# WeiZhang1988/YDORBSLAM

Measured on AMD Instinct MI355X. Metric: ORB extract+match Mkeypoints/sec, higher is better.
Workload: dtype u8

## Files before the change

### ydorbslam_amd/csrc/ba_kernels.hip.h

```cpp
#pragma once
#include <hip/hip_runtime.h>
#include <stdint.h>
#include "g2o_math.hip.h"

#pragma clang fp contract(off)

namespace ydorb {
namespace ba {

using g2o::R; using g2o::V3; using g2o::Q4;
using g2o::add; using g2o::cross; using g2o::scale; using g2o::qrot; using g2o::qmul; using g2o::qToR; using g2o::rToQ; using g2o::qnormalize;
using g2o::huber; using g2o::block_sums; using g2o::block_sum1; using g2o::dense_solve; using g2o::lambda_init; using g2o::lm_judge;

struct Cam { R fx, fy, cx, cy, bf; };

struct EdgeSoA {
  const int* pose;
  const int* pidx;
  const int* pt;
  const R* meas;
  const R* info;
  const uint8_t* robust;
  int n;
};
// ... 55 lines not shown
    for (int j = 0; j < 6; j++) B[2][j] = 0;
  }
}

__device__ __forceinline__ R block_sum(R v, R* lds) {
#pragma unroll
  for (int o = 32; o >= 1; o >>= 1) v += __shfl_xor(v, o, 64);
  const int lane = threadIdx.x & 63, wv = threadIdx.x >> 6, nw = blockDim.x >> 6;
  __syncthreads();
  if (lane == 0) lds[wv] = v;
  __syncthreads();
  R s = 0;
  for (int i = 0; i < nw; i++) s += lds[i];
  return s;
}

__device__ __forceinline__ void b_errors(EdgeSoA Ed, const R* __restrict__ poses, const R* __restrict__ pts, Cam cam,
                                                R deltaMono, R deltaStereo, R* __restrict__ err, R* __restrict__ partial) {
  __shared__ R lds[4];
  const int e = blockIdx.x * 256 + threadIdx.x;
  R chi = 0;
  if (e < Ed.n) {
    V3 t; Q4 q;
    load_pose(poses, Ed.pose[e], t, q);
    const R* X = pts + 3 * Ed.pt[e];
    const R* z = Ed.meas + 3 * e;
    const bool st = z[2] >= 0;
    R r[3], d;
    residual(t, q, V3{X[0], X[1], X[2]}, z, st, cam, r, &d);
    if (Ed.info[e] != 0) {
      err[3 * e] = r[0]; err[3 * e + 1] = r[1]; err[3 * e + 2] = r[2];
      const R c2 = Ed.info[e] * (r[0] * r[0] + r[1] * r[1] + r[2] * r[2]);
      if (Ed.robust[e]) { R r0, r1; huber(c2, st ? deltaStereo : deltaMono, &r0, &r1); chi = r0; }
      else chi = c2;
    }
  }
  const R s = block_sum(chi, lds);
  if (threadIdx.x == 0) partial[blockIdx.x] = s;
}
__global__ __launch_bounds__(256) void k_errors(EdgeSoA Ed, const R* __restrict__ poses, const R* __restrict__ pts, Cam cam,
                                                R deltaMono, R deltaStereo, R* __restrict__ err, R* __restrict__ partial) { b_errors(Ed, poses, pts, cam, deltaMono, deltaStereo, err, partial); }

__device__ __forceinline__ void b_sum_partials(const R* __restrict__ partial, int n, R* __restrict__ out, int slot,
                                                      const int* __restrict__ status) {
  __shared__ R lds[4];
  R v = 0;
  for (int i = threadIdx.x; i < n; i += 256) v += partial[i];
  const R s = block_sum(v, lds);
  if (threadIdx.x == 0) {
    out[slot] = s;
    if (status) { out[6] = (R)status[0]; out[7] = (R)status[1]; }
  }
}
__global__ __launch_bounds__(256) void k_sum_partials(const R* __restrict__ partial, int n, R* __restrict__ out, int slot,
                                                      const int* __restrict__ status) { b_sum_partials(partial, n, out, slot, status); }


__device__ __forceinline__ void b_build_points(EdgeSoA Ed, const int* __restrict__ ptStart, int nL, const R* __restrict__ poses,
                                                      const R* __restrict__ pts, Cam cam, R deltaMono, R deltaStereo,
                                                      const R* __restrict__ err, R* __restrict__ Hll, R* __restrict__ bl,
                                                      R* __restrict__ Hpl) {
  const int l = blockIdx.x * 128 + threadIdx.x;
  if (l >= nL) return;
  R h[6] = {0, 0, 0, 0, 0, 0}, b[3] = {0, 0, 0};
  for (int e = ptStart[l]; e < ptStart[l + 1]; e++) {
    const R w = Ed.info[e];
    if (w == 0) {
      if (Ed.pidx[e] >= 0)
        for (int k = 0; k < 18; k++) Hpl[(size_t)18 * e + k] = 0;
      continue;
    }
    V3 t; Q4 q;
    load_pose(poses, Ed.pose[e], t, q);
    const R* X = pts + 3 * Ed.pt[e];
    const bool st = Ed.meas[3 * e + 2] >= 0;
    R A[3][3], B[3][6];
    jacobians(t, q, V3{X[0], X[1], X[2]}, st, cam, A, B);
    const R r0 = err[3 * e], r1 = err[3 * e + 1], r2 = err[3 * e + 2];
    R rho1 = 1;
    if (Ed.robust[e]) { R rr; huber(w * (r0 * r0 + r1 * r1 + r2 * r2), st ? deltaStereo : deltaMono, &rr, &rho1); }
    const R W = rho1 * w;
    const R omr[3] = {-w * r0 * rho1, -w * r1 * rho1, -w * r2 * rho1};
    int k = 0;
#pragma unroll
    for (int r = 0; r < 3; r++)
#pragma unroll
      for (int c = r; c < 3; c++, k++) h[k] += A[0][r] * W * A[0][c] + A[1][r] * W * A[1][c] + A[2][r] * W * A[2][c];
#pragma unroll
    for (int r = 0; r < 3; r++) b[r] += A[0][r] * omr[0] + A[1][r] * omr[1] + A[2][r] * omr[2];
    if (Ed.pidx[e] >= 0) {
      R* hp = Hpl + (size_t)18 * e;
#pragma unroll
      for (int r = 0; r < 6; r++)
#pragma unroll
        for (int c = 0; c < 3; c++) hp[r * 3 + c] = B[0][r] * W * A[0][c] + B[1][r] * W * A[1][c] + B[2][r] * W * A[2][c];
    }
  }
#pragma unroll
  for (int k = 0; k < 6; k++) Hll[(size_t)6 * l + k] = h[k];
  bl[3 * l] = b[0]; bl[3 * l + 1] = b[1]; bl[3 * l + 2] = b[2];
}
__global__ __launch_bounds__(128) void k_build_points(EdgeSoA Ed, const int* __restrict__ ptStart, int nL, const R* __restrict__ poses,
                                                      const R* __restrict__ pts, Cam cam, R deltaMono, R deltaStereo,
                                                      const R* __restrict__ err, R* __restrict__ Hll, R* __restrict__ bl,
                                                      R* __restrict__ Hpl) { b_build_points(Ed, ptStart, nL, poses, pts, cam, deltaMono, deltaStereo, err, Hll, bl, Hpl); }


__device__ __forceinline__ void b_build_poses(EdgeSoA Ed, const int* __restrict__ poseStart, const int* __restrict__ poseEdges,
// ... 32 lines not shown
  }
  __shared__ R part[4][27];
  const int lane = threadIdx.x & 63, wv = threadIdx.x >> 6;
#pragma unroll
  for (int k = 0; k < 21; k++) {
#pragma unroll
    for (int o = 32; o >= 1; o >>= 1) h[k] += __shfl_xor(h[k], o, 64);
    if (lane == 0) part[wv][k] = h[k];
  }
#pragma unroll
  for (int k = 0; k < 6; k++) {
#pragma unroll
    for (int o = 32; o >= 1; o >>= 1) b[k] += __shfl_xor(b[k], o, 64);
    if (lane == 0) part[wv][21 + k] = b[k];
  }
  __syncthreads();
  if (threadIdx.x < 27) {
    const int k = threadIdx.x;
    const R sum = part[0][k] + part[1][k] + part[2][k] + part[3][k];
    if (k < 21) {
      int r = 0, rem = k;
      while (rem >= 6 - r) { rem -= 6 - r; r++; }
      const int c = r + rem;
      Hpp[(size_t)36 * i + r * 6 + c] = sum;
      Hpp[(size_t)36 * i + c * 6 + r] = sum;
    } else {
      bp[6 * i + (k - 21)] = sum;
    }
  }
  (void)lds;
}
__global__ __launch_bounds__(256) void k_build_poses(EdgeSoA Ed, const int* __restrict__ poseStart, const int* __restrict__ poseEdges,
                                                     const R* __restrict__ poses, const R* __restrict__ pts, Cam cam, R deltaMono,
                                                     R deltaStereo, const R* __restrict__ err, R* __restrict__ Hpp,
                                                     R* __restrict__ bp) { b_build_poses(Ed, poseStart, poseEdges, poses, pts, cam, deltaMono, deltaStereo, err, Hpp, bp); }


__device__ __forceinline__ void b_max_diag(const R* __restrict__ Hpp, int nP, const R* __restrict__ Hll, int nL, R* __restrict__ out,
                                                  int slot) {
  __shared__ R lds[4];
  R m = 0;
  for (int i = threadIdx.x; i < 6 * nP; i += 256) m = fmax(m, fabs(Hpp[(size_t)36 * (i / 6) + (i % 6) * 7]));
  for (int i = threadIdx.x; i < 3 * nL; i += 256) {
    const int l = i / 3, d = i % 3;
    m = fmax(m, fabs(Hll[(size_t)6 * l + (d == 0 ? 0 : d == 1 ? 3 : 5)]));
  }
#pragma unroll
  for (int o = 32; o >= 1; o >>= 1) m = fmax(m, __shfl_xor(m, o, 64));
  if ((threadIdx.x & 63) == 0) lds[threadIdx.x >> 6] = m;
  __syncthreads();
  if (threadIdx.x == 0) out[slot] = fmax(fmax(lds[0], lds[1]), fmax(lds[2], lds[3]));
}
__global__ __launch_bounds__(256) void k_max_diag(const R* __restrict__ Hpp, int nP, const R* __restrict__ Hll, int nL, R* __restrict__ out,
                                                  int slot) { b_max_diag(Hpp, nP, Hll, nL, out, slot); }


__device__ __forceinline__ void b_dinv(const R* __restrict__ Hll, const R* __restrict__ bl, int nL, R lambda, R* __restrict__ Dinv,
                                              R* __restrict__ db, int* __restrict__ status) {
  const int l = blockIdx.x * 256 + threadIdx.x;
  if (l == 0) { status[0] = 0; status[1] = 0; }
  if (l >= nL) return;
  const R* d = Hll + (size_t)6 * l;
  const R a = d[0] + lambda, b = d[1], c = d[2], e = d[3] + lambda, f = d[4], i = d[5] + lambda;
  const R c00 = e * i - f * f, c01 = c * f - b * i, c02 = b * f - c * e;
  const R id = 1.0 / (a * c00 + b * c01 + c * c02);
  R o[6] = {c00 * id, c01 * id, c02 * id, (a * i - c * c) * id, (b * c - a * f) * id, (a * e - b * b) * id};
#pragma unroll
  for (int k = 0; k < 6; k++) Dinv[(size_t)6 * l + k] = o[k];
  const R b0 = bl[3 * l], b1 = bl[3 * l + 1], b2 = bl[3 * l + 2];
  db[3 * l] = o[0] * b0 + o[1] * b1 + o[2] * b2;
  db[3 * l + 1] = o[1] * b0 + o[3] * b1 + o[4] * b2;
  db[3 * l + 2] = o[2] * b0 + o[4] * b1 + o[5] * b2;
}
__global__ __launch_bounds__(256) void k_dinv(const R* __restrict__ Hll, const R* __restrict__ bl, int nL, R lambda, R* __restrict__ Dinv,
                                              R* __restrict__ db, int* __restrict__ status) { b_dinv(Hll, bl, nL, lambda, Dinv, db, status); }


__device__ __forceinline__ int pair_bucket(int i1, int i2) { return i2 * (i2 + 1) / 2 + i1; }

__global__ __launch_bounds__(256) void k_pair_count(EdgeSoA Ed, const int* __restrict__ ptStart, int nL, int* __restrict__ cnt) {
  const int l = blockIdx.x * 256 + threadIdx.x;
  if (l >= nL) return;
  for (int a = ptStart[l]; a < ptStart[l + 1]; a++) {
    const int i1 = Ed.pidx[a];
    if (i1 < 0) continue;
    for (int b = a; b < ptStart[l + 1]; b++) {
      const int i2 = Ed.pidx[b];
      if (i2 >= 0) atomicAdd(&cnt[pair_bucket(i1, i2)], 1);
    }
  }
}
__global__ __launch_bounds__(256) void k_excl_scan(const int* __restrict__ in, int n, int* __restrict__ out) {
  __shared__ int wsum[4];
  __shared__ int carryS;
  const int lane = threadIdx.x & 63, wv = threadIdx.x >> 6;
  if (threadIdx.x == 0) carryS = 0;
  __syncthreads();
  for (int c0 = 0; c0 < n; c0 += 256) {
    const int i = c0 + threadIdx.x;
    const int v = i < n ? in[i] : 0;
    int x = v;
#pragma unroll
    for (int d = 1; d < 64; d <<= 1) { const int y = __shfl_up(x, d, 64); if (lane >= d) x += y; }
    if (lane == 63) wsum[wv] = x;
    __syncthreads();
    int off = carryS;
    for (int j = 0; j < wv; j++) off += wsum[j];
// ... 878 lines not shown
```

### ydorbslam_amd/csrc/ba_solver.hip

```cpp
#include <hip/hip_runtime.h>
#include <chrono>

#include <algorithm>
#include <functional>
#include <string>
#include <thread>
#include <atomic>
#include <cmath>
#include <cstring>
#include <limits>
#include <mutex>
#include <numeric>
#include <vector>

#include "../../include/ydorb/c_api.h"
#include "ba_kernels.hip.h"
#include "host_buffers.h"
#include "ydorb_host.h"

using namespace ydorb;
using namespace ydorb::ba;

namespace {

// ... 17 lines not shown

struct UpPtrs { int *ePose, *ePidx, *ePt, *eLm, *ptStart, *poseStart, *ptOf, *poseEdges, *poseOf; double *eMeas, *eInfo; uint8_t* eRobust; };
size_t layUp(const Sys& Y, void* base, UpPtrs& u) {
  Carve a(base);
  const size_t Ea = Y.Ea;
  a.take(u.ePose, Ea); a.take(u.ePidx, Ea); a.take(u.ePt, Ea); a.take(u.eLm, Ea); a.take(u.eMeas, 3 * Ea); a.take(u.eInfo, Ea); a.take(u.eRobust, Ea);
  a.take(u.ptStart, Y.nL + 1); a.take(u.poseStart, Y.nPf + 1); a.take(u.ptOf, Y.nL); a.take(u.poseEdges, Y.nPoseEdges); a.take(u.poseOf, Y.nPf);
  return a.L.bytes;
}

struct WorkPtrs {
  double *eInfo0, *err, *partial, *Hll, *bl, *Hpl, *BD, *Hpp, *S, *diagInv, *diagL, *Dinv, *db, *xp, *xl, *yv, *scal;
  uint8_t* eOutlier;
  int *status, *pairCnt, *pairStart, *pairCursor;
  int2 *pairA, *pairB;
  double* bp(const Sys& Y) const { return Hpp + (size_t)36 * Y.nPf; }
  double* bs(const Sys& Y) const { return S + (size_t)Y.n * Y.n; }
};
size_t layWork(const Sys& Y, void* base, WorkPtrs& w) {
  Carve a(base);
  const size_t Ea = Y.Ea, nL = Y.nL, nPf = Y.nPf, n = Y.n, tiles = (size_t)Y.nb * NB * NB, nBk = (size_t)Y.nBuckets + 1, items = std::max<size_t>(Y.nItems, 1);
  a.take(w.eInfo0, Ea); a.take(w.eOutlier, Ea); a.take(w.err, 3 * Ea); a.take(w.partial, Y.nBlkE + (6 * nPf + 3 * nL + 255) / 256 + 1);
  a.take(w.Hll, 6 * nL); a.take(w.bl, 3 * nL); a.take(w.Hpl, 18 * Ea); a.take(w.BD, 18 * Ea); a.take(w.Hpp, 42 * std::max<size_t>(nPf, 1));
  a.take(w.S, n * n + n + tiles); w.diagInv = w.S + n * n + n;
  a.take(w.diagL, tiles); a.take(w.Dinv, 6 * nL); a.take(w.db, 3 * nL); a.take(w.xp, n); a.take(w.yv, n); a.take(w.xl, 3 * nL);
  a.take(w.scal, 8); a.take(w.status, 2); a.take(w.pairCnt, nBk); a.take(w.pairStart, nBk); a.take(w.pairCursor, nBk); a.take(w.pairA, items); a.take(w.pairB, items);
  return a.L.bytes;
}

struct PosePtrs { int *start, *inl, *trials; double *poses, *X, *meas, *info, *err, *chi; uint8_t *flags, *outlier; };
size_t layPose(int n, size_t E, void* base, PosePtrs& q) {
  Carve a(base);
  a.take(q.start, n + 1); a.take(q.poses, (size_t)7 * n); a.take(q.X, 3 * E); a.take(q.meas, 3 * E); a.take(q.info, E);
  a.take(q.err, 3 * E); a.take(q.flags, E); a.take(q.outlier, E); a.take(q.inl, n); a.take(q.chi, (size_t)4 * n); a.take(q.trials, n);
  return a.L.bytes;
}

struct SolveMem {
  int device = -1;
  hipStream_t stream = nullptr;
  Mem state, up, work;
  StatePtrs st{};
  UpPtrs u{};
  WorkPtrs w{};
  PinnedMem hStage;
  int stage(size_t bytes) { return bytes <= hStage.cap ? YDORB_OK : hStage.alloc(bytes + bytes / 4 + 4096); }
  void releaseBuffers() { for (Mem* m : {&state, &up, &work, static_cast<Mem*>(&hStage)}) m->release(); }
};

struct Ctx {
  SolveMem mem;
  Mem pose;
  hipEvent_t ev[2 * PH_COUNT + 2]{};
  PinnedMem hPin;
  void releaseBuffers() { mem.releaseBuffers(); pose.release(); }
};
constexpr int kCtxPool = 8;
std::mutex g_mu[16][kCtxPool];
Ctx g_ctx[16][kCtxPool];
std::mutex g_pick;

Ctx* acquireCtx(int device, std::unique_lock<std::mutex>& lock) {
  int slot = -1;
  {
    std::lock_guard<std::mutex> pick(g_pick);
    for (int i = 0; i < kCtxPool && slot < 0; i++)
      if (g_mu[device][i].try_lock()) slot = i;
  }
  if (slot < 0) { slot = 0; g_mu[device][0].lock(); }
  lock = std::unique_lock<std::mutex>(g_mu[device][slot], std::adopt_lock);
  Ctx& c = g_ctx[device][slot];
  auto init = [&]() -> int {
    c.mem.device = device;
    HIPCHK(hipStreamCreateWithFlags(&c.mem.stream, hipStreamNonBlocking));
    for (auto& e : c.ev) HIPCHK(hipEventCreate(&e));
    return c.hPin.alloc(sizeof(double) * 16);
  };
  if (!c.mem.stream && init() != YDORB_OK) return nullptr;
  return &c;
}

struct Run {
  SolveMem* c;
  const YdBaProblem* P;
  const YdBaOptions* O;
  YdBaResult* res;
  int cur = 0;
  bool noRobust = false;
  Cam cam;
  bool phaseTimes = false;
  double phaseMs[PH_COUNT] = {0, 0, 0, 0, 0};
  bool pending[PH_COUNT] = {false, false, false, false, false};
  Sys sys;
  hipEvent_t* ev = nullptr;
  double* hPin = nullptr;
  bool stopped() const { return P->stop && *P->stop; }
};

int allreduce(Run& R_, void* d_buf, int64_t count, int op) {
  const YdBaOptions* O = R_.O;
  if (!O->allreduce || O->world <= 1) return YDORB_OK;
  if (count > O->comm_doubles || !O->d_comm_buf) { set_error("BA comm buffer too small (%lld doubles needed)", (long long)count); return YDORB_ERR_CAPACITY; }
  HIPCHK(hipMemcpyAsync(O->d_comm_buf, d_buf, sizeof(double) * count, hipMemcpyDeviceToDevice, R_.c->stream));
  HIPCHK(hipStreamSynchronize(R_.c->stream));
  if (O->allreduce(O->allreduce_user, O->d_comm_buf, count, op) != 0) { set_error("BA all-reduce callback failed"); return YDORB_ERR_HIP; }
  HIPCHK(hipMemcpyAsync(d_buf, O->d_comm_buf, sizeof(double) * count, hipMemcpyDeviceToDevice, R_.c->stream));
  return YDORB_OK;
}

static bool g_trace = getenv("YDORB_BA_TRACE") != nullptr && getenv("YDORB_BA_TRACE")[0] == '1';
static std::chrono::steady_clock::time_point g_t0;
static void trace(const char* what) {
  if (!g_trace) return;
  fprintf(stderr, "[ba %8.3f ms] %s\n", std::chrono::duration<double, std::milli>(std::chrono::steady_clock::now() - g_t0).count(), what);
}

struct PhaseTimer {
  Run& r; int ph; hipEvent_t a, b; bool on;
  PhaseTimer(Run& r_, int ph_) : r(r_), ph(ph_), a(r_.ev[2 * ph_]), b(r_.ev[2 * ph_ + 1]), on(r_.phaseTimes) {
    if (!on) return;
    collect(r_, ph_);
    (void)hipEventRecord(a, r.c->stream);
  }
  void stop() { if (on) { (void)hipEventRecord(b, r.c->stream); on = false; r.pending[ph] = true; } }
  static void collect(Run& r_, int ph_) {
    if (!r_.pending[ph_]) return;
    float ms = 0;
    if (hipEventSynchronize(r_.ev[2 * ph_ + 1]) == hipSuccess && hipEventElapsedTime(&ms, r_.ev[2 * ph_], r_.ev[2 * ph_ + 1]) == hipSuccess)
      r_.phaseMs[ph_] += ms;
    r_.pending[ph_] = false;
  }
};

int prepareStage(Run& R_, bool reuse) {
  SolveMem& c = *R_.c;
  const YdBaProblem& P = *R_.P;
  const YdBaOptions& O = *R_.O;
  hipStream_t s = c.stream;
  const int K = P.n_poses, NP = P.n_points, E = P.n_edges;
  trace("optimize: begin");
  Sys& Y = R_.sys;
  auto prepare = [&]() -> int {
    std::vector<int> act;
    for (int e = 0; e < E; e++) act.push_back(e);
    if (act.empty()) { Y.Ea = 0; return YDORB_OK; }
    std::vector<int> poseIdx(K, -1), ptIdx(NP, -1), poseOf, ptOf;
    {
      std::vector<uint8_t> pu(K, 0), qu(NP, 0);
      for (int e : act) { pu[P.edge_pose[e]] = 1; qu[P.edge_point[e]] = 1; }
      for (int k = 0; k < K; k++) if (pu[k] && !P.pose_fixed[k]) { poseIdx[k] = (int)poseOf.size(); poseOf.push_back(k); }
      for (int p = 0; p < NP; p++) if (qu[p]) { ptIdx[p] = (int)ptOf.size(); ptOf.push_back(p); }
    }
    const int nL = (int)ptOf.size(), Ea = (int)act.size();
    if (O.world > 1) {
      poseOf.clear();
      for (int k = 0; k < K; k++) { poseIdx[k] = -1; if (!P.pose_fixed[k]) { poseIdx[k] = (int)poseOf.size(); poseOf.push_back(k); } }
    }
    const int nPf = (int)poseOf.size();
    {
// ... 54 lines not shown
      };
      auto upv = [&](const auto* dst, const auto& vec) { up(dst, vec.data(), sizeof(vec[0]) * vec.size()); };
      upv(u.ePose, hPose); upv(u.ePidx, hPidx); upv(u.ePt, hPt); upv(u.eLm, hLm); upv(u.eMeas, hMeas); upv(u.eInfo, hInfo);
      upv(u.eRobust, hRobust); upv(u.ptStart, hPtStart); upv(u.poseStart, hPoseStart); upv(u.ptOf, ptOf);
      upv(u.poseEdges, hPoseEdges); upv(u.poseOf, poseOf);
      HIPCHK(hipMemcpyAsync(c.up.p, c.hStage.p, upBytes, hipMemcpyHostToDevice, s));
      HIPCHK(hipMemcpyAsync(w.eInfo0, u.eInfo, sizeof(double) * Ea, hipMemcpyDeviceToDevice, s));
      HIPCHK(hipMemsetAsync(w.err, 0, sizeof(double) * 3 * Ea, s));
    }
    trace("optimize: uploads enqueued");
    if (Z.nBuckets > 0) {
      const int nBuckets = Z.nBuckets;
      EdgeSoA Ed{u.ePose, u.ePidx, u.ePt, u.eMeas, u.eInfo, u.eRobust, Ea};
      HIPCHK(hipMemsetAsync(w.pairCnt, 0, sizeof(int) * (nBuckets + 1), s));
      hipLaunchKernelGGL(k_pair_count, dim3((nL + 255) / 256), dim3(256), 0, s, Ed, u.ptStart, nL, w.pairCnt);
      hipLaunchKernelGGL(k_excl_scan, dim3(1), dim3(256), 0, s, w.pairCnt, nBuckets, w.pairStart);
      HIPCHK(hipMemcpyAsync(w.pairCursor, w.pairStart, sizeof(int) * (nBuckets + 1), hipMemcpyDeviceToDevice, s));
      hipLaunchKernelGGL(k_pair_fill, dim3((nL + 255) / 256), dim3(256), 0, s, Ed, u.ptStart, nL, w.pairCursor, w.pairA);
      hipLaunchKernelGGL(k_pair_sort, dim3((nBuckets + 3) / 4), dim3(256), 0, s, w.pairStart, nBuckets, w.pairA, w.pairB);
    }
    HIPCHK(hipStreamSynchronize(s));
    Z.act.swap(act);
    Y = std::move(Z);
    return YDORB_OK;
  };
  int rc;
  if (!reuse || Y.Ea == 0) {
    if ((rc = prepare())) return rc;
  }
  if (Y.Ea == 0) return YDORB_OK;
  HIPCHK(hipMemcpyAsync(c.st.poses[R_.cur ^ 1], c.st.poses[R_.cur], sizeof(double) * 7 * K, hipMemcpyDeviceToDevice, s));
  HIPCHK(hipMemcpyAsync(c.st.pts[R_.cur ^ 1], c.st.pts[R_.cur], sizeof(double) * 3 * NP, hipMemcpyDeviceToDevice, s));
  HIPCHK(hipMemsetAsync(c.w.S, 0, sizeof(double) * ((size_t)Y.n * Y.n + Y.n + (size_t)Y.nb * NB * NB), s));
  return YDORB_OK;
}

int optimize(Run& R_, int iterations, int stage, bool reuse) {
  int rc = prepareStage(R_, reuse);
  if (rc) return rc;
  SolveMem& c = *R_.c;
  const YdBaOptions& O = *R_.O;
  hipStream_t s = c.stream;
  const Sys& Y = R_.sys;
  if (Y.Ea == 0) return YDORB_OK;
  const int nL = Y.nL, nPf = Y.nPf, Ea = Y.Ea, n = Y.n, nb = Y.nb, nBlkE = Y.nBlkE, nBuckets = Y.nBuckets;
  const UpPtrs& u = c.u;
  const WorkPtrs& w = c.w;
  double* const* poses = c.st.poses;
  double* const* pts = c.st.pts;
  double *dHpp = w.Hpp, *dbp = w.bp(Y), *dS = w.S, *dbs = w.bs(Y);
  EdgeSoA Ed{u.ePose, u.ePidx, u.ePt, u.eMeas, u.eInfo, u.eRobust, Ea};
  const double dM = O.delta_mono, dSt = O.delta_stereo;
  double* hscal = R_.hPin;
  int* hstatus = reinterpret_cast<int*>(R_.hPin + 8);
  const bool multi = O.world > 1 && O.allreduce;

  auto computeChi2 = [&](int buf, double* out, bool withStatus) -> int {
    PhaseTimer t(R_, PH_ERR);
    hipLaunchKernelGGL(k_errors, dim3(nBlkE), dim3(256), 0, s, Ed, poses[buf], pts[buf], R_.cam, dM, dSt, w.err, w.partial);
    hipLaunchKernelGGL(k_sum_partials, dim3(1), dim3(256), 0, s, w.partial, nBlkE, w.scal, 0, withStatus ? w.status : nullptr);
    t.stop();
    if (multi) { int r2 = allreduce(R_, w.scal, 1, 0); if (r2) return r2; }
    HIPCHK(hipMemcpyAsync(hscal, w.scal, sizeof(double) * 8, hipMemcpyDeviceToHost, s));
    HIPCHK(hipStreamSynchronize(s));
    if (withStatus) { hstatus[0] = (int)hscal[6]; hstatus[1] = (int)hscal[7]; }
    *out = hscal[0];
    return YDORB_OK;
  };

  trace("optimize: pair buckets enqueued");
  double lambda = 0, ni = 2, currentChi = 0;
  bool lastAccepted = true;
  for (int it = 0; it < iterations && !R_.stopped(); it++) {
    if ((it == 0 || !lastAccepted) && (rc = computeChi2(R_.cur, &currentChi, false))) return rc;
    {
      PhaseTimer t(R_, PH_BUILD);
      hipLaunchKernelGGL(k_build_points, dim3((nL + 127) / 128), dim3(128), 0, s, Ed, u.ptStart, nL, poses[R_.cur], pts[R_.cur], R_.cam, dM, dSt, w.err, w.Hll, w.bl, w.Hpl);
      if (nPf)
        hipLaunchKernelGGL(k_build_poses, dim3(nPf), dim3(256), 0, s, Ed, u.poseStart, u.poseEdges, poses[R_.cur], pts[R_.cur], R_.cam, dM, dSt, w.err, dHpp, dbp);
      t.stop();
      if (multi && nPf) { if ((rc = allreduce(R_, dHpp, (int64_t)42 * nPf, 0))) return rc; }
    }
    if (it == 0) {
      hipLaunchKernelGGL(k_max_diag, dim3(1), dim3(256), 0, s, dHpp, nPf, w.Hll, nL, w.scal, 1);
      if (multi) { if ((rc = allreduce(R_, w.scal + 1, 1, 1))) return rc; }
      HIPCHK(hipMemcpyAsync(hscal, w.scal, sizeof(double) * 8, hipMemcpyDeviceToHost, s));
      HIPCHK(hipStreamSynchronize(s));
      lambda = 1e-5 * hscal[1];
      ni = 2;
    }
    double rho = 0;
    int qmax = 0;
    do {
      const int nxt = R_.cur ^ 1;
      {
        PhaseTimer t(R_, PH_SCHUR);
        const double contrib = (!multi || O.rank == 0) ? 1.0 : 0.0;
        hipLaunchKernelGGL(k_dinv, dim3((nL + 255) / 256), dim3(256), 0, s, w.Hll, w.bl, nL, lambda, w.Dinv, w.db, w.status);
        hipLaunchKernelGGL(k_bd, dim3(nBlkE), dim3(256), 0, s, Ed, u.eLm, w.Hpl, w.Dinv, w.BD);
        if (nPf)
          hipLaunchKernelGGL(k_bs, dim3(nPf), dim3(256), 0, s, Ed, u.poseStart, u.poseEdges, u.eLm, w.Hpl, w.db, dbp, contrib, dbs);
        hipLaunchKernelGGL(k_schur_pairs, dim3(nBuckets + 1), dim3(64 * kSchurWaves), 0, s, w.pairStart, w.pairB, nPf, nBuckets, w.BD, w.Hpl, dHpp, lambda, contrib, n, dS, dbs);
        t.stop();
      }
      if (multi) {
        if ((rc = allreduce(R_, dS, (int64_t)n * n + n, 0))) return rc;
      }
      {
        PhaseTimer t(R_, PH_SOLVE);
        for (int kb = 0; kb < nb; kb++)
          hipLaunchKernelGGL(k_chol_step, dim3((nb - kb) * (nb - kb + 1) / 2 + (kb > 0)), dim3(256), 0, s, dS, w.diagL, w.diagInv, n, kb, w.status, dbs, w.yv);
        if (!launch_chol_solve(s, dS, w.diagInv, n, w.yv, dbs, w.xp)) {
          set_error("reduced camera system of %d rows is wider than the solve kernel's LDS (max %d)", n, kCholSolveMaxN);
          return YDORB_ERR_UNSUPPORTED;
        }
        hipLaunchKernelGGL(k_backsub, dim3((nL + 127) / 128), dim3(128), 0, s, Ed, u.ptStart, nL, w.Hpl, w.Dinv, w.bl, w.xp, w.xl);
        t.stop();
        HIPCHK(hipGetLastError());
      }
      {
        PhaseTimer t(R_, PH_UPDATE);
        hipLaunchKernelGGL(k_update, dim3((std::max(nPf, nL) + 255) / 256), dim3(256), 0, s, poses[R_.cur], pts[R_.cur], poses[nxt], pts[nxt], u.poseOf, nPf, u.ptOf, nL, w.xp, w.xl);
        {
          const int np6 = (!multi || O.rank == 0) ? 6 * nPf : 0;
          const int nb2 = (np6 + 3 * nL + 255) / 256;
          hipLaunchKernelGGL(k_scale, dim3(nb2), dim3(256), 0, s, w.xp, dbp, np6, w.xl, w.bl, 3 * nL, lambda, w.partial + nBlkE);
          hipLaunchKernelGGL(k_sum_partials, dim3(1), dim3(256), 0, s, w.partial + nBlkE, nb2, w.scal, 2, nullptr);
        }
        t.stop();
        if (multi) { if ((rc = allreduce(R_, w.scal + 2, 1, 0))) return rc; }
      }
      double tempChi;
      if ((rc = computeChi2(nxt, &tempChi, true))) return rc;
      const double scaleSum = hscal[2];
      lastAccepted = lm_judge(lambda, ni, currentChi, rho, tempChi, scaleSum + 1e-3, hstatus[0] == 0);
      if (lastAccepted) R_.cur = nxt;
      else if (!std::isfinite(lambda)) { qmax++; R_.res->n_trials++; break; }
      qmax++;
      R_.res->n_trials++;
    } while (rho < 0 && qmax < O.max_trials && !R_.stopped());
    YdBaResult* res = R_.res;
    if (res->n_log < 32) {
      res->log_chi2[res->n_log] = currentChi; res->log_lambda[res->n_log] = lambda; res->log_trials[res->n_log] = qmax; res->log_stage[res->n_log] = stage;
      res->n_log++;
    }
    res->n_iterations++;
    if (qmax == O.max_trials || rho == 0 || !std::isfinite(lambda)) break;
  }
  trace("optimize: LM loop done");
  for (int ph = 0; ph < PH_COUNT; ph++) PhaseTimer::collect(R_, ph);
  trace("optimize: errors read back");
  return YDORB_OK;
}

int checkProblem(const YdBaProblem* P, const YdBaOptions* optIn, YdBaResult* res, YdBaOptions* Oout) {
  if (!P || !res) { set_error("null argument"); return YDORB_ERR_INVALID_ARG; }
  YdBaOptions O;
  if (optIn) O = *optIn; else ydorb_ba_default_options(&O);
  uint8_t* outlier = res->edge_outlier;
  memset(res, 0, sizeof(*res));
  res->edge_outlier = outlier;
  const int K = P->n_poses, NP = P->n_points, E = P->n_edges;
  if (K < 0 || NP < 0 || E < 0 || (K && (!P->poses || !P->pose_fixed)) || (NP && !P->points) ||
      (E && (!P->edge_pose || !P->edge_point || !P->edge_meas || !P->edge_inv_sigma2)) || O.device < 0 || O.device >= 16 || O.max_trials < 1) {
    set_error("invalid BA problem");
    return YDORB_ERR_INVALID_ARG;
  }
  for (int e = 0; e < E; e++)
    if (P->edge_pose[e] < 0 || P->edge_pose[e] >= K || P->edge_point[e] < 0 || P->edge_point[e] >= NP) {
      set_error("edge %d references a vertex out of range", e);
      return YDORB_ERR_INVALID_ARG;
    }
  if (outlier) memset(outlier, 0, E);
  *Oout = O;
  return YDORB_OK;
}

int beginSolve(Run& R_) {
  SolveMem& c = *R_.c;
  const YdBaProblem* P = R_.P;
// ... 180 lines not shown
        }
        if (!r) {
          startStage(j, 1);
          r = X.rc;
        }
        if (r) { X.errText = ydorb_last_error(); fail(j, r); }
        if (hipStreamSynchronize(st) != hipSuccess && !r) { X.errText = "hipStreamSynchronize failed"; fail(j, YDORB_ERR_HIP); }
        X.mem.stream = s;
      }
    };
    std::vector<std::thread> pool;
    for (int t = 1; t < nt; t++) pool.emplace_back(worker, t);
    worker(0);
    for (std::thread& th : pool) th.join();
    for (int j = 0; j < n; j++) if (J[j]->rc != YDORB_OK) set_error("%s", J[j]->errText.c_str());
  }
  trace("batch: set-up done");

  auto maxOver = [&](auto fn) { int m = 0; for (int j = 0; j < n; j++) if (!J[j]->done) m = std::max(m, fn(J[j]->run->sys)); return m; };
  auto rounds = [&]() -> int {
  while (true) {
    bool any = false;
    for (int j = 0; j < n; j++) any = any || !J[j]->done;
    if (!any) break;
    trace("batch: round begins");
    bool anyBuild = false, anyChi = false, anyDiag = false;
    for (int j = 0; j < n; j++) {
      Job& X = *J[j];
      BaDev& D = hDev[j];
      D.trial = 0;
      D.build = !X.done && X.needBuild;
      D.chi2 = D.build && (X.it == 0 || !X.lastAccepted);
      D.maxdiag = D.build && X.it == 0;
      D.cur = X.done ? 0 : X.run->cur;
      D.lambda = X.lambda;
      anyBuild = anyBuild || D.build; anyChi = anyChi || D.chi2; anyDiag = anyDiag || D.maxdiag;
    }
    const int gE = maxOver([](const Sys& Y) { return Y.nBlkE; }), gL128 = maxOver([](const Sys& Y) { return (Y.nL + 127) / 128; }),
              gL256 = maxOver([](const Sys& Y) { return (Y.nL + 255) / 256; }), gP = maxOver([](const Sys& Y) { return Y.nPf; }),
              gBk = maxOver([](const Sys& Y) { return Y.nBuckets + 1; }), gNb = maxOver([](const Sys& Y) { return Y.nb; }),
              gUpd = maxOver([](const Sys& Y) { return (std::max(Y.nPf, Y.nL) + 255) / 256; }),
              gScale = maxOver([](const Sys& Y) { return (6 * Y.nPf + 3 * Y.nL + 255) / 256; }), gN = maxOver([](const Sys& Y) { return Y.n; });
    const BaDev* dDev = B.dDev.as<BaDev>();
    if (anyBuild) {
      HIPCHK(hipMemcpyAsync(B.dDev.p, hDev, sizeof(BaDev) * n, hipMemcpyHostToDevice, s));
      if (anyChi) {
        hipLaunchKernelGGL(kb_errors, dim3(gE, 1, n), dim3(256), 0, s, dDev, 0);
        hipLaunchKernelGGL(kb_sum_partials, dim3(1, 1, n), dim3(256), 0, s, dDev, 0);
      }
      hipLaunchKernelGGL(kb_build_points, dim3(gL128, 1, n), dim3(128), 0, s, dDev);
      if (gP) hipLaunchKernelGGL(kb_build_poses, dim3(gP, 1, n), dim3(256), 0, s, dDev);
      if (anyDiag) hipLaunchKernelGGL(kb_max_diag, dim3(1, 1, n), dim3(256), 0, s, dDev);
      HIPCHK(hipGetLastError());
      if (anyChi || anyDiag) {
        HIPCHK(hipMemcpyAsync(hScal, dScalAll, sizeof(double) * 8 * n, hipMemcpyDeviceToHost, s));
        HIPCHK(hipStreamSynchronize(s));
      }
      for (int j = 0; j < n; j++) {
        Job& X = *J[j];
        const BaDev& D = hDev[j];
        if (!D.build) continue;
        if (D.chi2) X.currentChi = hScal[8 * j + 0];
        if (D.maxdiag) { X.lambda = 1e-5 * hScal[8 * j + 1]; X.ni = 2; }
        X.needBuild = false;
      }
    }
    for (int j = 0; j < n; j++) {
      Job& X = *J[j];
      BaDev& D = hDev[j];
      D.build = D.chi2 = D.maxdiag = 0;
      D.trial = !X.done;
      D.lambda = X.lambda;
      D.cur = X.done ? 0 : X.run->cur;
    }
    HIPCHK(hipMemcpyAsync(B.dDev.p, hDev, sizeof(BaDev) * n, hipMemcpyHostToDevice, s));
    hipLaunchKernelGGL(kb_dinv, dim3(gL256, 1, n), dim3(256), 0, s, dDev);
    hipLaunchKernelGGL(kb_bd, dim3(gE, 1, n), dim3(256), 0, s, dDev);
    if (gP) hipLaunchKernelGGL(kb_bs, dim3(gP, 1, n), dim3(256), 0, s, dDev);
    hipLaunchKernelGGL(kb_schur_pairs, dim3(gBk, 1, n), dim3(64 * kSchurWaves), 0, s, dDev);
    for (int kb = 0; kb < gNb; kb++)
      hipLaunchKernelGGL(kb_chol_step, dim3((gNb - kb) * (gNb - kb + 1) / 2 + (kb > 0), 1, n), dim3(256), 0, s, dDev, kb);
    {
      const size_t dyn = sizeof(double) * (size_t)gN;
      if (dyn > 48 * 1024)
        HIPCHK(hipFuncSetAttribute(reinterpret_cast<const void*>(kb_chol_solve), hipFuncAttributeMaxDynamicSharedMemorySize, (int)dyn));
      hipLaunchKernelGGL(kb_chol_solve, dim3(1, 1, n), dim3(1024), dyn, s, dDev);
    }
    hipLaunchKernelGGL(kb_backsub, dim3(gL128, 1, n), dim3(128), 0, s, dDev);
    hipLaunchKernelGGL(kb_update, dim3(gUpd, 1, n), dim3(256), 0, s, dDev);
    hipLaunchKernelGGL(kb_scale, dim3(gScale, 1, n), dim3(256), 0, s, dDev);
    hipLaunchKernelGGL(kb_sum_partials, dim3(1, 1, n), dim3(256), 0, s, dDev, 2);
    hipLaunchKernelGGL(kb_errors, dim3(gE, 1, n), dim3(256), 0, s, dDev, 1);
    hipLaunchKernelGGL(kb_sum_partials, dim3(1, 1, n), dim3(256), 0, s, dDev, 1);
    HIPCHK(hipGetLastError());
    HIPCHK(hipMemcpyAsync(hScal, dScalAll, sizeof(double) * 8 * n, hipMemcpyDeviceToHost, s));
    HIPCHK(hipStreamSynchronize(s));
    trace("batch: round synchronised");
    for (int j = 0; j < n; j++) {
      Job& X = *J[j];
      if (X.done) continue;
      const double* hs = hScal + (size_t)8 * j;
      const double tempChi = hs[0], scaleSum = hs[2];
      X.lastAccepted = lm_judge(X.lambda, X.ni, X.currentChi, X.rho, tempChi, scaleSum + 1e-3, (int)hs[6] == 0);
      if (X.lastAccepted) X.run->cur ^= 1;
      const bool lambdaBroke = !X.lastAccepted && !std::isfinite(X.lambda);
      X.qmax++;
      X.run->res->n_trials++;
      if (lambdaBroke || !(X.rho < 0 && X.qmax < X.O.max_trials && !X.run->stopped())) endIteration(j);
    }
  }
  return YDORB_OK;
  };
  {
    int rr = rounds();
    if (rr == YDORB_OK && hipStreamSynchronize(s) != hipSuccess) { set_error("hipStreamSynchronize failed after the lock-step rounds"); rr = YDORB_ERR_HIP; }
    if (rr != YDORB_OK) {
      const std::string text = ydorb_last_error();
      for (int j = 0; j < n; j++)
        if (J[j]->rc == YDORB_OK && J[j]->run && (!J[j]->done || J[j]->pendingEnd)) { J[j]->pendingEnd = false; J[j]->errText = text; fail(j, rr); }
      set_error("%s", text.c_str());
      return rr;
    }
  }
  {
    const int nt = std::max(1, std::min(n, (int)B.setupStreams.size()));
    std::atomic<int> next{0};
    auto worker = [&](int t) {
      (void)hipSetDevice(Oin.device);
      for (int j = next.fetch_add(1); j < n; j = next.fetch_add(1)) {
        Job& X = *J[j];
        if (!X.pendingEnd) continue;
        X.pendingEnd = false;
        X.mem.stream = B.setupStreams[t];
        const int r = endSolve(*X.run);
        X.mem.stream = s;
        if (r) { X.errText = ydorb_last_error(); fail(j, r); }
      }
    };
    std::vector<std::thread> pool;
    for (int t = 1; t < nt; t++) pool.emplace_back(worker, t);
    worker(0);
    for (std::thread& th : pool) th.join();
    for (int j = 0; j < n; j++) if (J[j]->rc != YDORB_OK && !J[j]->errText.empty()) set_error("%s", J[j]->errText.c_str());
  }
  trace("batch: done");
  int first = YDORB_OK;
  for (int j = 0; j < n; j++) if (J[j]->rc != YDORB_OK && first == YDORB_OK) first = J[j]->rc;
  return first;
}

}

extern "C" {

void ydorb_ba_default_options(YdBaOptions* o) {
  if (!o) return;
  memset(o, 0, sizeof(*o));
  o->iters1 = 5; o->iters2 = 10;
  o->chi2_mono = 5.991; o->chi2_stereo = 7.815;
  o->delta_mono = (double)(float)sqrt(5.991);
  o->delta_stereo = (double)(float)sqrt(7.815);
  o->max_trials = 10;
  o->device = 0;
  o->rank = 0; o->world = 1;
}

int ydorb_ba_solve(const YdBaProblem* P, const YdBaOptions* optIn, YdBaResult* res) {
  YdBaOptions O;
  int rc = checkProblem(P, optIn, res, &O);
  if (rc) return rc;
  const int K = P->n_poses, NP = P->n_points, E = P->n_edges;
  if (P->stop && *P->stop) { res->stopped = 1; return YDORB_OK; }
  if (E == 0 || K == 0 || NP == 0) return YDORB_OK;
  if ((rc = require_device(O.device))) return rc;
  g_t0 = std::chrono::steady_clock::now();
  trace("solve: begin");
  std::unique_lock<std::mutex> lock;
  Ctx* ctx = acquireCtx(O.device, lock);
  if (!ctx) return YDORB_ERR_HIP;
  Ctx& c = *ctx;
  Run R_{&c.mem, P, &O, res};
  R_.ev = c.ev; R_.hPin = c.hPin.as<double>();
  if ((rc = beginSolve(R_))) return rc;
  trace("solve: state uploaded");
  hipEvent_t t0 = c.ev[2 * PH_COUNT], t1 = c.ev[2 * PH_COUNT + 1];
  HIPCHK(hipEventRecord(t0, c.mem.stream));

  if ((rc = optimize(R_, O.iters1, 1, false))) return rc;
  if (O.flags & YDORB_BA_SINGLE_STAGE) {
  } else if (!R_.stopped()) {
    if ((rc = cullAfterFirstStage(R_))) return rc;
    trace("solve: depths read");
    if ((rc = optimize(R_, O.iters2, 2, true))) return rc;
  } else {
    res->stopped = 1;
  }
  HIPCHK(hipEventRecord(t1, c.mem.stream));
  if ((rc = endSolve(R_))) return rc;
  (void)hipEventElapsedTime(&res->ms_total, t0, t1);
  trace("solve: results read back");
  res->ms_errors = (float)R_.phaseMs[PH_ERR]; res->ms_build = (float)R_.phaseMs[PH_BUILD]; res->ms_schur = (float)R_.phaseMs[PH_SCHUR];
  res->ms_solve = (float)R_.phaseMs[PH_SOLVE]; res->ms_update = (float)R_.phaseMs[PH_UPDATE];
  return YDORB_OK;
}

int ydorb_pose_optimize(const YdPoseBatch* B, uint8_t* outlier, int32_t* n_inliers, double* chi2_log, int32_t* trials) {
  if (!B || B->n_frames < 0 || (B->n_frames && (!B->edge_start || !B->poses || !n_inliers)) || B->device < 0 || B->device >= 16) {
    set_error("invalid pose batch");
    return YDORB_ERR_INVALID_ARG;
  }
  const int n = B->n_frames;
  if (n == 0) return YDORB_OK;
  if (B->edge_start[0] != 0) { set_error("edge_start[0] must be 0"); return YDORB_ERR_INVALID_ARG; }
  for (int f = 0; f < n; f++)
    if (B->edge_start[f + 1] < B->edge_start[f]) { set_error("edge_start must be non-decreasing"); return YDORB_ERR_INVALID_ARG; }
  const int E = B->edge_start[n];
  if (E > 0 && (!B->points || !B->meas || !B->inv_sigma2 || !outlier)) { set_error("null edge arrays"); return YDORB_ERR_INVALID_ARG; }
  int rc = require_device(B->device);
  if (rc) return rc;
  std::unique_lock<std::mutex> lock;
  Ctx* c = acquireCtx(B->device, lock);
  if (!c) return YDORB_ERR_HIP;
  hipStream_t s = c->mem.stream;
  const size_t Ez = (size_t)std::max(E, 1);
  PosePtrs q;
  if ((rc = c->pose.ensure(layPose(n, Ez, nullptr, q)))) return rc;
  layPose(n, Ez, c->pose.p, q);
  HIPCHK(hipMemcpyAsync(q.start, B->edge_start, sizeof(int) * (n + 1), hipMemcpyHostToDevice, s));
  HIPCHK(hipMemcpyAsync(q.poses, B->poses, sizeof(double) * 7 * n, hipMemcpyHostToDevice, s));
  if (E) {
    HIPCHK(hipMemcpyAsync(q.X, B->points, sizeof(double) * 3 * E, hipMemcpyHostToDevice, s));
    HIPCHK(hipMemcpyAsync(q.meas, B->meas, sizeof(double) * 3 * E, hipMemcpyHostToDevice, s));
    HIPCHK(hipMemcpyAsync(q.info, B->inv_sigma2, sizeof(double) * E, hipMemcpyHostToDevice, s));
  }
  const Cam cam{B->fx, B->fy, B->cx, B->cy, B->bf};
// ... 112 lines not shown
```

### ydorbslam_amd/csrc/host_buffers.h

```cpp
#pragma once
#include <hip/hip_runtime.h>

#include <algorithm>
#include <cstddef>
#include <cstdint>
#include <mutex>

#include "../../include/ydorb/c_api.h"
#include "ydorb_host.h"

#define HIPCHK(expr)                                                                          \
  do {                                                                                        \
    hipError_t _e = (expr);                                                                   \
    if (_e != hipSuccess) {                                                                   \
      ydorb::set_error("%s failed: %s (%s:%d)", #expr, hipGetErrorString(_e), __FILE__, __LINE__); \
      return YDORB_ERR_HIP;                                                                   \
    }                                                                                         \
  } while (0)

namespace ydorb {

struct Mem {
  void* p = nullptr;
  size_t cap = 0;
  bool host = false;
  size_t slackDiv = 4, floor = 4096;
  size_t want(size_t bytes) const { return std::max(bytes + bytes / slackDiv, floor); }
  int ensure(size_t bytes) { return bytes <= cap ? YDORB_OK : alloc(want(bytes)); }
  int alloc(size_t bytes) {
    release();
    if ((host ? hipHostMalloc(&p, bytes) : hipMalloc(&p, bytes)) != hipSuccess) {
      p = nullptr;
      set_error("%s(%zu) failed", host ? "hipHostMalloc" : "hipMalloc", bytes);
      return YDORB_ERR_HIP;
    }
    cap = bytes;
    return YDORB_OK;
  }
  void release() {
    if (p) (void)(host ? hipHostFree(p) : hipFree(p));
    p = nullptr; cap = 0;
  }
  void take(Mem& o) { release(); p = o.p; cap = o.cap; o.p = nullptr; o.cap = 0; }
  template <class T> T* as() { return reinterpret_cast<T*>(p); }
  template <class T> T* at(size_t off) { return reinterpret_cast<T*>(static_cast<uint8_t*>(p) + off); }
};

struct PinnedMem : Mem {
  PinnedMem() { host = true; }
};

struct ScopedMem : Mem {
  ScopedMem() = default;
  ScopedMem(const ScopedMem&) = delete;
  ScopedMem& operator=(const ScopedMem&) = delete;
  ~ScopedMem() { release(); }
};

template <class T> T* at(Mem& m, size_t off) { return m.at<T>(off); }

struct Layout {
  size_t bytes = 0, align = 16;
  size_t add(size_t n) { const size_t at = bytes; bytes += (n + align - 1) & ~(align - 1); return at; }
};

struct StagedCtx {
  std::mutex mu;
  hipStream_t stream = nullptr;
  Mem up, down, scratch;
  PinnedMem hUp, hDown;
  int init(int device) {
    HIPCHK(hipSetDevice(device));
    if (!stream) HIPCHK(hipStreamCreateWithFlags(&stream, hipStreamNonBlocking));
    return YDORB_OK;
  }
  void releaseBuffers() { up.release(); down.release(); scratch.release(); hUp.release(); hDown.release(); }
};

inline int release_staged(StagedCtx& c, int device) {
  std::lock_guard<std::mutex> lock(c.mu);
  HIPCHK(hipSetDevice(device));
  if (c.stream) (void)hipStreamSynchronize(c.stream);
  c.releaseBuffers();
  return YDORB_OK;
}

}
```

Baseline: 182.8.

## Publish BA scalars to mapped host memory and poll instead of memcpy+sync

The reduction kernels (k_sum_partials, k_max_diag) now write the scalar results plus a sequence number straight into coherent, mapped pinned host memory using system-scope atomic stores. The host spin-polls that sequence word for up to a set budget before falling back to the old async memcpy plus stream synchronize. The aim is to cut the D2H copy and sync latency on every LM iteration of the single-GPU solve. In exchange the host burns CPU while spinning, and correctness rests on ordering between the system fence and the sequence store.

```diff
diff --git a/ydorbslam_amd/csrc/ba_kernels.hip.h b/ydorbslam_amd/csrc/ba_kernels.hip.h
--- a/ydorbslam_amd/csrc/ba_kernels.hip.h
+++ b/ydorbslam_amd/csrc/ba_kernels.hip.h
@@ -131,8 +131,22 @@
     if (status) { out[6] = (R)status[0]; out[7] = (R)status[1]; }
   }
 }
+
+__device__ __forceinline__ void publish_scal(const R* scal, R* mapped, unsigned long long seq) {
+  if (!mapped || threadIdx.x != 0) return;
+  R v[8];
+#pragma unroll
+  for (int i = 0; i < 8; i++) v[i] = scal[i];
+#pragma unroll
+  for (int i = 0; i < 8; i++) __hip_atomic_store(mapped + i, v[i], __ATOMIC_RELAXED, __HIP_MEMORY_SCOPE_SYSTEM);
+  __threadfence_system();
+  __hip_atomic_store(reinterpret_cast<unsigned long long*>(mapped + 8), seq, __ATOMIC_RELAXED, __HIP_MEMORY_SCOPE_SYSTEM);
+}
 __global__ __launch_bounds__(256) void k_sum_partials(const R* __restrict__ partial, int n, R* __restrict__ out, int slot,
-                                                      const int* __restrict__ status) { b_sum_partials(partial, n, out, slot, status); }
+                                                      const int* __restrict__ status, R* mapped, unsigned long long seq) {
+  b_sum_partials(partial, n, out, slot, status);
+  publish_scal(out, mapped, seq);
+}
 
 
 __device__ __forceinline__ void b_build_points(EdgeSoA Ed, const int* __restrict__ ptStart, int nL, const R* __restrict__ poses,
@@ -271,7 +285,10 @@
   if (threadIdx.x == 0) out[slot] = fmax(fmax(lds[0], lds[1]), fmax(lds[2], lds[3]));
 }
 __global__ __launch_bounds__(256) void k_max_diag(const R* __restrict__ Hpp, int nP, const R* __restrict__ Hll, int nL, R* __restrict__ out,
-                                                  int slot) { b_max_diag(Hpp, nP, Hll, nL, out, slot); }
+                                                  int slot, R* mapped, unsigned long long seq) {
+  b_max_diag(Hpp, nP, Hll, nL, out, slot);
+  publish_scal(out, mapped, seq);
+}
 
 
 __device__ __forceinline__ void b_dinv(const R* __restrict__ Hll, const R* __restrict__ bl, int nL, R lambda, R* __restrict__ Dinv,
diff --git a/ydorbslam_amd/csrc/ba_solver.hip b/ydorbslam_amd/csrc/ba_solver.hip
--- a/ydorbslam_amd/csrc/ba_solver.hip
+++ b/ydorbslam_amd/csrc/ba_solver.hip
@@ -93,10 +93,13 @@
   SolveMem mem;
   Mem pose;
   hipEvent_t ev[2 * PH_COUNT + 2]{};
-  PinnedMem hPin;
+  PinnedMem hPin{PinnedMem::kDeviceWrites};
+  double* dPin = nullptr;
+  uint64_t seq = 0;
   void releaseBuffers() { mem.releaseBuffers(); pose.release(); }
 };
 constexpr int kCtxPool = 8;
+constexpr long kPollBudgetUs = 2000;
 std::mutex g_mu[16][kCtxPool];
 Ctx g_ctx[16][kCtxPool];
 std::mutex g_pick;
@@ -115,7 +118,10 @@
     c.mem.device = device;
     HIPCHK(hipStreamCreateWithFlags(&c.mem.stream, hipStreamNonBlocking));
     for (auto& e : c.ev) HIPCHK(hipEventCreate(&e));
-    return c.hPin.alloc(sizeof(double) * 16);
+    int rc = c.hPin.alloc(sizeof(double) * 16);
+    if (rc) return rc;
+    memset(c.hPin.p, 0, sizeof(double) * 16);
+    return c.hPin.devicePtr(reinterpret_cast<void**>(&c.dPin));
   };
   if (!c.mem.stream && init() != YDORB_OK) return nullptr;
   return &c;
@@ -135,6 +141,9 @@
   Sys sys;
   hipEvent_t* ev = nullptr;
   double* hPin = nullptr;
+  double* dPin = nullptr;
+  uint64_t* seq = nullptr;
+  long pollUs = 0;
   bool stopped() const { return P->stop && *P->stop; }
 };
 
@@ -146,6 +155,13 @@
   HIPCHK(hipStreamSynchronize(R_.c->stream));
   if (O->allreduce(O->allreduce_user, O->d_comm_buf, count, op) != 0) { set_error("BA all-reduce callback failed"); return YDORB_ERR_HIP; }
   HIPCHK(hipMemcpyAsync(d_buf, O->d_comm_buf, sizeof(double) * count, hipMemcpyDeviceToDevice, R_.c->stream));
+  return YDORB_OK;
+}
+
+int readScal(hipStream_t s, double* host, const double* dev, size_t count, const volatile uint64_t* seqWord, uint64_t expect, long budgetUs) {
+  if (seqWord && poll_sequence(seqWord, expect, budgetUs)) return YDORB_OK;
+  HIPCHK(hipMemcpyAsync(host, dev, sizeof(double) * count, hipMemcpyDeviceToHost, s));
+  HIPCHK(hipStreamSynchronize(s));
   return YDORB_OK;
 }
 
@@ -306,17 +322,21 @@
   EdgeSoA Ed{u.ePose, u.ePidx, u.ePt, u.eMeas, u.eInfo, u.eRobust, Ea};
   const double dM = O.delta_mono, dSt = O.delta_stereo;
   double* hscal = R_.hPin;
-  int* hstatus = reinterpret_cast<int*>(R_.hPin + 8);
+  const volatile uint64_t* hseq = reinterpret_cast<const uint64_t*>(R_.hPin + 8);
+  int* hstatus = reinterpret_cast<int*>(R_.hPin + 9);
   const bool multi = O.world > 1 && O.allreduce;
+  double* const dPub = multi ? nullptr : R_.dPin;
+  auto nextSeq = [&]() -> unsigned long long { return dPub ? ++*R_.seq : 0; };
+  auto readBack = [&]() -> int { return readScal(s, hscal, w.scal, 8, dPub ? hseq : nullptr, *R_.seq, R_.pollUs); };
 
   auto computeChi2 = [&](int buf, double* out, bool withStatus) -> int {
     PhaseTimer t(R_, PH_ERR);
     hipLaunchKernelGGL(k_errors, dim3(nBlkE), dim3(256), 0, s, Ed, poses[buf], pts[buf], R_.cam, dM, dSt, w.err, w.partial);
-    hipLaunchKernelGGL(k_sum_partials, dim3(1), dim3(256), 0, s, w.partial, nBlkE, w.scal, 0, withStatus ? w.status : nullptr);
+    hipLaunchKernelGGL(k_sum_partials, dim3(1), dim3(256), 0, s, w.partial, nBlkE, w.scal, 0, withStatus ? w.status : nullptr, dPub, nextSeq());
     t.stop();
-    if (multi) { int r2 = allreduce(R_, w.scal, 1, 0); if (r2) return r2; }
-    HIPCHK(hipMemcpyAsync(hscal, w.scal, sizeof(double) * 8, hipMemcpyDeviceToHost, s));
-    HIPCHK(hipStreamSynchronize(s));
+    int r2;
+    if (multi && (r2 = allreduce(R_, w.scal, 1, 0))) return r2;
+    if ((r2 = readBack())) return r2;
     if (withStatus) { hstatus[0] = (int)hscal[6]; hstatus[1] = (int)hscal[7]; }
     *out = hscal[0];
     return YDORB_OK;
@@ -336,10 +356,9 @@
       if (multi && nPf) { if ((rc = allreduce(R_, dHpp, (int64_t)42 * nPf, 0))) return rc; }
     }
     if (it == 0) {
-      hipLaunchKernelGGL(k_max_diag, dim3(1), dim3(256), 0, s, dHpp, nPf, w.Hll, nL, w.scal, 1);
+      hipLaunchKernelGGL(k_max_diag, dim3(1), dim3(256), 0, s, dHpp, nPf, w.Hll, nL, w.scal, 1, dPub, nextSeq());
       if (multi) { if ((rc = allreduce(R_, w.scal + 1, 1, 1))) return rc; }
-      HIPCHK(hipMemcpyAsync(hscal, w.scal, sizeof(double) * 8, hipMemcpyDeviceToHost, s));
-      HIPCHK(hipStreamSynchronize(s));
+      if ((rc = readBack())) return rc;
       lambda = 1e-5 * hscal[1];
       ni = 2;
     }
@@ -379,7 +398,7 @@
           const int np6 = (!multi || O.rank == 0) ? 6 * nPf : 0;
           const int nb2 = (np6 + 3 * nL + 255) / 256;
           hipLaunchKernelGGL(k_scale, dim3(nb2), dim3(256), 0, s, w.xp, dbp, np6, w.xl, w.bl, 3 * nL, lambda, w.partial + nBlkE);
-          hipLaunchKernelGGL(k_sum_partials, dim3(1), dim3(256), 0, s, w.partial + nBlkE, nb2, w.scal, 2, nullptr);
+          hipLaunchKernelGGL(k_sum_partials, dim3(1), dim3(256), 0, s, w.partial + nBlkE, nb2, w.scal, 2, nullptr, nullptr, 0ull);
         }
         t.stop();
         if (multi) { if ((rc = allreduce(R_, w.scal + 2, 1, 0))) return rc; }
@@ -666,10 +685,8 @@
       if (gP) hipLaunchKernelGGL(kb_build_poses, dim3(gP, 1, n), dim3(256), 0, s, dDev);
       if (anyDiag) hipLaunchKernelGGL(kb_max_diag, dim3(1, 1, n), dim3(256), 0, s, dDev);
       HIPCHK(hipGetLastError());
-      if (anyChi || anyDiag) {
-        HIPCHK(hipMemcpyAsync(hScal, dScalAll, sizeof(double) * 8 * n, hipMemcpyDeviceToHost, s));
-        HIPCHK(hipStreamSynchronize(s));
-      }
+      int rb;
+      if ((anyChi || anyDiag) && (rb = readScal(s, hScal, dScalAll, (size_t)8 * n, nullptr, 0, 0))) return rb;
       for (int j = 0; j < n; j++) {
         Job& X = *J[j];
         const BaDev& D = hDev[j];
@@ -707,8 +724,8 @@
     hipLaunchKernelGGL(kb_errors, dim3(gE, 1, n), dim3(256), 0, s, dDev, 1);
     hipLaunchKernelGGL(kb_sum_partials, dim3(1, 1, n), dim3(256), 0, s, dDev, 1);
     HIPCHK(hipGetLastError());
-    HIPCHK(hipMemcpyAsync(hScal, dScalAll, sizeof(double) * 8 * n, hipMemcpyDeviceToHost, s));
-    HIPCHK(hipStreamSynchronize(s));
+    int rb;
+    if ((rb = readScal(s, hScal, dScalAll, (size_t)8 * n, nullptr, 0, 0))) return rb;
     trace("batch: round synchronised");
     for (int j = 0; j < n; j++) {
       Job& X = *J[j];
@@ -795,6 +812,13 @@
   Ctx& c = *ctx;
   Run R_{&c.mem, P, &O, res};
   R_.ev = c.ev; R_.hPin = c.hPin.as<double>();
+  {
+    const char* mode = getenv("YDORB_BA_READBACK");
+    const char* us = getenv("YDORB_BA_POLL_US");
+    R_.dPin = mode && !strcmp(mode, "sync") ? nullptr : c.dPin;
+    R_.seq = &c.seq;
+    R_.pollUs = us && *us ? atol(us) : kPollBudgetUs;
+  }
   if ((rc = beginSolve(R_))) return rc;
   trace("solve: state uploaded");
   hipEvent_t t0 = c.ev[2 * PH_COUNT], t1 = c.ev[2 * PH_COUNT + 1];
diff --git a/ydorbslam_amd/csrc/host_buffers.h b/ydorbslam_amd/csrc/host_buffers.h
--- a/ydorbslam_amd/csrc/host_buffers.h
+++ b/ydorbslam_amd/csrc/host_buffers.h
@@ -2,6 +2,8 @@
 #include <hip/hip_runtime.h>
 
 #include <algorithm>
+#include <atomic>
+#include <chrono>
 #include <cstddef>
 #include <cstdint>
 #include <mutex>
@@ -24,12 +26,13 @@
   void* p = nullptr;
   size_t cap = 0;
   bool host = false;
+  unsigned hostFlags = hipHostMallocDefault;
   size_t slackDiv = 4, floor = 4096;
   size_t want(size_t bytes) const { return std::max(bytes + bytes / slackDiv, floor); }
   int ensure(size_t bytes) { return bytes <= cap ? YDORB_OK : alloc(want(bytes)); }
   int alloc(size_t bytes) {
     release();
-    if ((host ? hipHostMalloc(&p, bytes) : hipMalloc(&p, bytes)) != hipSuccess) {
+    if ((host ? hipHostMalloc(&p, bytes, hostFlags) : hipMalloc(&p, bytes)) != hipSuccess) {
       p = nullptr;
       set_error("%s(%zu) failed", host ? "hipHostMalloc" : "hipMalloc", bytes);
       return YDORB_ERR_HIP;
@@ -47,8 +50,28 @@
 };
 
 struct PinnedMem : Mem {
-  PinnedMem() { host = true; }
+  static constexpr unsigned kDeviceWrites = hipHostMallocMapped | hipHostMallocCoherent;
+  explicit PinnedMem(unsigned flags = hipHostMallocDefault) { host = true; hostFlags = flags; }
+  int devicePtr(void** out) {
+    *out = nullptr;
+    HIPCHK(hipHostGetDevicePointer(out, p, 0));
+    return YDORB_OK;
+  }
 };
+
+inline bool poll_sequence(const volatile uint64_t* word, uint64_t expect, long budgetUs) {
+  if (budgetUs <= 0) return false;
+  const auto deadline = std::chrono::steady_clock::now() + std::chrono::microseconds(budgetUs);
+  for (;;) {
+    for (int i = 0; i < 256; i++) {
+      if (*word == expect) { std::atomic_thread_fence(std::memory_order_acquire); return true; }
+#if defined(__x86_64__) && !defined(__HIP_DEVICE_COMPILE__)
+      __builtin_ia32_pause();
+#endif
+    }
+    if (std::chrono::steady_clock::now() >= deadline) return false;
+  }
+}
 
 struct ScopedMem : Mem {
   ScopedMem() = default;
```

Measured after the change: 182.8. Within noise of the previous version (-0.0%).
